# sim590/opendht

Measured on AMD Instinct MI355X. Metric: k=8 closest-node queries/sec at 100M-node table (1/8 GPU) + % HBM roofline, higher is better.
Workload: dtype u64

## Files before the change

opendht_amd/csrc/kad_swarm.hip:

```cpp
#include <hip/hip_runtime.h>

#include <algorithm>
#include <cstdlib>
#include <cstdarg>
#include <cstdint>
#include <cstdio>
#include <cstring>
#include <mutex>
#include <string>
#include <vector>

#include "../../include/kadgpu.h"

namespace kadgpu_internal {
int set_error(int code, const char* msg);
bool device_ok(int dev);
}

namespace {

constexpr uint32_t NONE = 0xFFFFFFFFu;
constexpr uint32_t L = KAD_SWARM_LEVELS;
constexpr uint32_t BK = 8;
constexpr uint32_t SN = 14;
// ... 197 lines not shown
    };
    const uint32_t lv = (uint32_t)(__builtin_bitreverse64(k) & ((1ull << D) - 1));
    const uint32_t m1 = lv, m0 = ~lv & (uint32_t)((1ull << D) - 1);
    const uint32_t M = (uint32_t)__builtin_popcount(m1), B = D + 1;
    const uint64_t x = k ^ t.hi;
    const uint32_t c = x ? (uint32_t)__builtin_clzll(x) : 64u;
    uint32_t b;
    if (c >= D) b = M;
    else if ((m1 >> c) & 1u) b = (uint32_t)__builtin_popcount(m1 & ((1u << c) - 1u));
    else b = M + 1 + (uint32_t)__builtin_popcount(m0 & ~((2u << c) - 1u));
    const uint32_t n0 = (uint32_t)__builtin_popcount(m0);
    auto level = [&](uint32_t P) -> uint32_t {
        if (P < M) return nth_bit(m1, P);
        if (P == M) return D;
        return nth_bit(m0, n0 - 1 - (P - M - 1));
    };
    uint32_t lo = b > 0 ? b - 1 : 0, hi = b, good = cnt(level(b)) + (b > 0 ? cnt(level(b - 1)) : 0u);
    while (good < count && !(lo == 0 && hi == B - 1)) {
        if (hi < B - 1) { hi++; good += cnt(level(hi)); }
        if (lo > 0) { lo--; good += cnt(level(lo)); }
    }
    uint64_t L0[K];
    uint32_t LI[K];
#pragma unroll
    for (uint32_t s = 0; s < K; s++) { L0[s] = ~0ull; LI[s] = NONE; }
    uint32_t nl = 0;
    uint64_t nin = ~0ull;
    bool tie = false;
    static_assert(!NET || K == BK, "the network ranks 8");
    static_assert(BK == 8, "a level's slots are four 16-byte key loads and one 16-byte index rule");
    struct Slots {
        uint64_t k[BK];
        uint4 rule;
        uint32_t nb;
    };
    auto load_level = [&](uint32_t P, Slots& S) {
        const uint32_t d = level(P);
        S.nb = cnt(d);
        const uint4* kp4 = reinterpret_cast<const uint4*>(W.lvl + ((size_t)p * L + d) * LVL_WORDS);
        S.rule = kp4[LVL_RULE / 4];
#pragma unroll
        for (int x = 0; x < 4; x++) {
            const uint4 u = kp4[x];
            S.k[2 * x] = ((uint64_t)u.y << 32) | u.x;
            S.k[2 * x + 1] = ((uint64_t)u.w << 32) | u.z;
        }
    };
    Slots cur, nxt;
    load_level(lo, cur);
    for (uint32_t P = lo; P <= hi; P++) {
        if (P < hi) load_level(P + 1, nxt);
        const uint32_t nb = cur.nb;
        const uint64_t* ek = cur.k;
        if constexpr (NET) {
            uint32_t ej[BK];
#pragma unroll
            for (uint32_t j = 0; j < BK; j++) {
                cur.k[j] = j < nb ? cur.k[j] ^ t.hi : ~0ull;
                ej[j] = j;
                tie |= j < nb && cur.k[j] == ~0ull;
            }
            sort8_kid(cur.k, ej);
#pragma unroll
            for (uint32_t s = 0; s < K; s++) {
                const bool sw = cur.k[K - 1 - s] < L0[s];
                nin = min(nin, sw ? L0[s] : cur.k[K - 1 - s]);
                L0[s] = sw ? cur.k[K - 1 - s] : L0[s];
                LI[s] = sw ? (cur.k[K - 1 - s] != ~0ull ? lvl_index(cur.rule, ej[K - 1 - s]) : NONE) : LI[s];
            }
#pragma unroll
            for (uint32_t h = K / 2; h >= 1; h >>= 1)
#pragma unroll
                for (uint32_t r = 0; r < K; r++)
                    if ((r & h) == 0) cx_kid(L0[r], LI[r], L0[r + h], LI[r + h]);
            nl = min(nl + nb, K);
            if (P < hi) cur = nxt;
            continue;
        }
        uint32_t ei[BK];
#pragma unroll
        for (uint32_t j = 0; j < BK; j++) ei[j] = lvl_index(cur.rule, j);
#pragma unroll 1
        for (uint32_t j = 0; j < nb; j++) {
            uint64_t cd = ek[0];
            uint32_t ci = ei[0];
#pragma unroll
            for (uint32_t y = 1; y < BK; y++) {
                cd = j == y ? ek[y] : cd;
                ci = j == y ? ei[y] : ci;
            }
            cd ^= t.hi;
            bool sh = false;
#pragma unroll
            for (uint32_t s = 0; s < K; s++) {
                const bool lt = sh || s >= nl || cd < L0[s] || (cd == L0[s] && tail_less(W, t, ci, LI[s]));
                sh = lt;
                const uint64_t n0_ = lt ? L0[s] : cd;
                const uint32_t n1_ = lt ? LI[s] : ci;
                if (lt) { L0[s] = cd; LI[s] = ci; }
                cd = n0_;
                ci = n1_;
            }
            nl = min(nl + 1, K);
        }
        if (P < hi) cur = nxt;
    }
    if constexpr (NET) {
#pragma unroll
        for (uint32_t s = 0; s + 1 < K; s++) tie |= L0[s] != ~0ull && L0[s] == L0[s + 1];
        tie |= nin != ~0ull && L0[K - 1] == nin;
        if (tie) return TIE;
    }
    const uint32_t m = min(nl, count);
#pragma unroll
    for (uint32_t s = 0; s < K; s++) {
        oi[s] = LI[s];
        ok[s] = L0[s] ^ t.hi;
    }
    return m;
}

__global__ __launch_bounds__(BLOCK) void swarm_closest_kernel(SwarmDev W, const uint32_t* peers, const uint8_t* targets, uint32_t q, uint32_t count,
                                     uint32_t* out_idx, uint8_t* out_cnt) {
    const uint32_t i = blockIdx.x * BLOCK + threadIdx.x;
    if (i >= q) return;
    uint32_t oi[SNP];
    uint64_t ok[SNP];
    const uint32_t p = peers[i];
    const uint32_t m = p < W.n ? peer_closest<SNP>(W, p, load_tgt(targets, i), count, oi, ok) : 0u;
    for (uint32_t s = 0; s < count; s++) out_idx[(size_t)i * count + s] = s < m ? oi[s] : NONE;
    if (out_cnt) out_cnt[i] = (uint8_t)m;
}

struct SearchDev {
    const uint32_t* src;
    const uint8_t* targets;
    uint32_t* li;
    uint64_t* lk;
    uint8_t* lq;
    uint8_t* lb;
    uint8_t* ln;
    uint32_t* hops;
    uint8_t* done;
    uint32_t* sel;
    uint32_t* ri;
    uint64_t* rk;
    uint8_t* rn;
    uint32_t* active;
    uint32_t* overflow;
    uint32_t* xo;
    uint8_t* xn;
    uint32_t S;
    uint32_t offline;
};

__device__ __forceinline__ uint64_t sw_mix(uint64_t x) {
    x += 0x9E3779B97F4A7C15ull;
    x = (x ^ (x >> 30)) * 0xBF58476D1CE4E5B9ull;
    x = (x ^ (x >> 27)) * 0x94D049BB133111EBull;
    return x ^ (x >> 31);
}

__device__ __forceinline__ bool swarm_offline(uint32_t p, uint32_t per10k) {
    return per10k && (uint32_t)(sw_mix((uint64_t)p * 0x9E37ull + 0xBADull) % 10000ull) < per10k;
}

__device__ __forceinline__ uint32_t lo_mask(uint32_t n) { return n >= 32 ? ~0u : (1u << n) - 1u; }

template <uint32_t N>
__device__ __forceinline__ void select_next(const SearchDev& X, uint32_t s, uint32_t n, uint32_t& qm, uint32_t bm,
                                            const uint32_t (&li)[N]) {
    uint32_t rest = ~(qm | bm) & lo_mask(min(n, N)), pick = 0;
#pragma unroll
    for (uint32_t a = 0; a < ALPHA; a++) {
        pick |= rest & (0u - rest);
        rest &= rest - 1u;
    }
    qm |= pick;
    uint32_t sel[ALPHA] = {NONE, NONE, NONE, NONE};
#pragma unroll
    for (uint32_t j = 0; j < N; j++) {
        const uint32_t rk = (uint32_t)__builtin_popcount(pick & ((1u << j) - 1u));
        if ((pick >> j) & 1u)
#pragma unroll
            for (uint32_t a = 0; a < ALPHA; a++)
                if (a == rk) sel[a] = li[j];
    }
    reinterpret_cast<uint4*>(X.sel)[s] = make_uint4(sel[0], sel[1], sel[2], sel[3]);
    if (!pick) X.done[s] = 2;
}

__device__ __forceinline__ uint32_t load_flags(const uint8_t* f, uint32_t s, uint32_t n = LST) {
    const uint4* p = reinterpret_cast<const uint4*>(f + (size_t)s * LST);
    uint32_t m = 0;
#pragma unroll
    for (int x = 0; x < (int)LST / 16; x++) {
        const uint4 u = 16u * x < n ? p[x] : make_uint4(0, 0, 0, 0);
        const uint32_t w[4] = {u.x, u.y, u.z, u.w};
#pragma unroll
        for (int y = 0; y < 4; y++)
#pragma unroll
            for (int z = 0; z < 4; z++) m |= (((w[y] >> (8 * z)) & 255u) ? 1u : 0u) << (16 * x + 4 * y + z);
    }
    return m;
}
__device__ __forceinline__ void store_flags(uint8_t* f, uint32_t s, uint32_t m, uint32_t n, uint32_t w = LST) {
    m &= lo_mask(n);
    uint4* p = reinterpret_cast<uint4*>(f + (size_t)s * LST);
#pragma unroll
    for (int x = 0; x < (int)LST / 16; x++) {
        if (16u * x >= w) continue;
        uint32_t w[4];
#pragma unroll
        for (int y = 0; y < 4; y++) {
            w[y] = 0;
#pragma unroll
            for (int z = 0; z < 4; z++) w[y] |= ((m >> (16 * x + 4 * y + z)) & 1u) << (8 * z);
        }
        p[x] = make_uint4(w[0], w[1], w[2], w[3]);
    }
}
static_assert(LST == 32 && ALPHA == 4, "the flag masks are 32 bits, the selection one 16-byte store");

__global__ __launch_bounds__(BLOCK) void search_init_kernel(SwarmDev W, SearchDev X) {
    const uint32_t s = blockIdx.x * BLOCK + threadIdx.x;
    if (s >= X.S) return;
    uint32_t li[SNP];
    uint64_t lk[SNP];
    uint32_t qm = 0;
    const uint32_t p = X.src[s];
    const uint32_t n = p < W.n ? peer_closest<SNP>(W, p, load_tgt(X.targets, s), SN, li, lk) : 0u;
    X.done[s] = n ? 0 : 2;
    X.hops[s] = 0;
    X.ln[s] = (uint8_t)n;
    if (n) select_next(X, s, n, qm, 0u, li);
#pragma unroll
    for (uint32_t j = 0; j < LST; j++) {
        X.li[(size_t)s * LST + j] = j < SNP && j < n ? li[j < SNP ? j : 0] : NONE;
        X.lk[(size_t)s * LST + j] = j < SNP && j < n ? lk[j < SNP ? j : 0] : ~0ull;
    }
    store_flags(X.lq, s, qm, n);
    store_flags(X.lb, s, 0u, n);
}

template <bool NET>
__global__ __launch_bounds__(BLOCK) __attribute__((amdgpu_waves_per_eu(SW_QUERY_WPE, 8))) void search_query_kernel(SwarmDev W, SearchDev X) {
    const uint32_t g = blockIdx.x * BLOCK + threadIdx.x;
    if (g >= X.S * ALPHA) return;
    const uint32_t s = g / ALPHA;
    const uint32_t sv = X.sel[g];
    const Tgt t = load_tgt(X.targets, s);
    const uint32_t v = X.done[s] ? NONE : sv;
    uint32_t oi[BK];
    uint64_t ok[BK];
    const bool up = v < W.n && !swarm_offline(v, X.offline);
    uint32_t m = up ? (NET ? peer_closest<BK, true>(W, v, t, BK, oi, ok) : TIE) : 0u;
    if (m == TIE) m = peer_closest<BK>(W, v, t, BK, oi, ok);
    if (m) {
        uint4* pi = reinterpret_cast<uint4*>(X.ri + (size_t)g * BK);
        uint4* pk = reinterpret_cast<uint4*>(X.rk + (size_t)g * BK);
#pragma unroll
        for (uint32_t x = 0; x < BK / 4; x++)
            if (4 * x < m) pi[x] = make_uint4(oi[4 * x], oi[4 * x + 1], oi[4 * x + 2], oi[4 * x + 3]);
#pragma unroll
        for (uint32_t x = 0; x < BK / 2; x++)
            if (2 * x < m)
                pk[x] = make_uint4((uint32_t)ok[2 * x], (uint32_t)(ok[2 * x] >> 32), (uint32_t)ok[2 * x + 1],
                                   (uint32_t)(ok[2 * x + 1] >> 32));
    }
    X.rn[g] = (uint8_t)m;
}

constexpr uint32_t XO_CAP = 64;

template <uint32_t N>
__device__ __forceinline__ void search_insert(const SwarmDev& W, const Tgt& t, uint32_t (&li)[N], uint64_t (&ld)[N],
                                              uint32_t& qm, uint32_t& bm, uint32_t& n, uint32_t r, uint64_t rd, bool rbad,
                                              bool& ovf) {
    bool found = false, anyeq = false;
    uint32_t pos = 0;
#pragma unroll
    for (uint32_t k = 0; k < N; k++) {
        if (k < n) {
            found |= li[k] == r;
            pos += ld[k] < rd;
            anyeq |= ld[k] == rd;
        }
    }
    if (found) return;
    uint32_t tie = 0;
    if (anyeq) {
#pragma unroll
        for (uint32_t k = 0; k < N; k++)
            if (k < n) tie |= (ld[k] == rd && li[k] != r ? 1u : 0u) << k;
    }
    while (tie) {
        const uint32_t k = (uint32_t)__builtin_ctz(tie);
        tie &= tie - 1u;
        uint32_t lk = 0;
#pragma unroll
        for (uint32_t x = 0; x < N; x++) lk = x == k ? li[x] : lk;
        pos += tail_less(W, t, lk, r);
    }
    uint32_t bad = (uint32_t)__builtin_popcount(bm & lo_mask(n));
    const bool full = n - bad >= SN;
    if (full) {
        uint32_t good = ~bm & lo_mask(n);
#pragma unroll
        for (uint32_t k = 0; k < SN; k++) good &= good - 1u;
        const uint32_t tt = good ? (uint32_t)__builtin_ctz(good) : n;
        n = tt;
        bad = (uint32_t)__builtin_popcount(bm & lo_mask(n));
        if (pos >= tt) return;
    }
    if (n == N) {
        bad -= (bm >> (N - 1)) & 1u;
        n--;
        ovf = true;
        if (pos >= n) return;
    }
#pragma unroll
    for (uint32_t k = N - 1; k > 0; k--) {
        li[k] = k > pos ? li[k - 1] : k == pos ? r : li[k];
        ld[k] = k > pos ? ld[k - 1] : k == pos ? rd : ld[k];
    }
    li[0] = pos == 0 ? r : li[0];
    ld[0] = pos == 0 ? rd : ld[0];
    const uint32_t low = lo_mask(pos), bit = 1u << pos;
    qm = (qm & low) | ((qm & ~low) << 1);
    bm = (bm & low) | ((bm & ~low) << 1) | (rbad ? bit : 0u);
    n++;
    bad += rbad ? 1u : 0u;
    if (n - bad > SN) {
        uint32_t good = ~bm & lo_mask(n);
#pragma unroll
        for (uint32_t k = 0; k < SN; k++) good &= good - 1u;
        n = (uint32_t)__builtin_ctz(good);
        bad = (uint32_t)__builtin_popcount(bm & lo_mask(n));
    }
}

struct Answers {
    uint32_t r[BK];
    uint64_t k[BK];
};
__device__ __forceinline__ void load_answers(const SearchDev& X, uint32_t g, uint32_t rn, Answers& A) {
    const uint4* pi = reinterpret_cast<const uint4*>(X.ri + (size_t)g * BK);
    const uint4* pk = reinterpret_cast<const uint4*>(X.rk + (size_t)g * BK);
#pragma unroll
    for (uint32_t x = 0; x < BK / 4; x++) {
        const uint4 u = 4 * x < rn ? pi[x] : make_uint4(NONE, NONE, NONE, NONE);
        A.r[4 * x] = u.x; A.r[4 * x + 1] = u.y; A.r[4 * x + 2] = u.z; A.r[4 * x + 3] = u.w;
    }
#pragma unroll
    for (uint32_t x = 0; x < BK / 2; x++) {
        const uint4 u = 2 * x < rn ? pk[x] : make_uint4(0, 0, 0, 0);
        A.k[2 * x] = ((uint64_t)u.y << 32) | u.x;
        A.k[2 * x + 1] = ((uint64_t)u.w << 32) | u.z;
    }
}

template <uint32_t N, bool FUSED>
__device__ __forceinline__ bool merge_lookup(const SwarmDev& W, const SearchDev& X, uint32_t s, uint32_t n0, uint32_t bm0,
                                             uint32_t xn) {
    {
        const Tgt t = load_tgt(X.targets, s);
        uint32_t li[N];
        uint64_t ld[N];
        uint32_t n = n0;
        const uint4 sv = reinterpret_cast<const uint4*>(X.sel)[s];
        const uint32_t sel[ALPHA] = {sv.x, sv.y, sv.z, sv.w};
        const uint32_t rn4 = FUSED ? 0u : *reinterpret_cast<const uint32_t*>(X.rn + (size_t)s * ALPHA);
        Answers A[2];
        if (!FUSED) load_answers(X, s * ALPHA, rn4 & 255u, A[0]);
        {
            const uint4* pi = reinterpret_cast<const uint4*>(X.li + (size_t)s * LST);
            const uint4* pk = reinterpret_cast<const uint4*>(X.lk + (size_t)s * LST);
#pragma unroll
            for (uint32_t x = 0; x < N / 4; x++) {
                const uint4 u = 4 * x < n0 ? pi[x] : make_uint4(NONE, NONE, NONE, NONE);
                li[4 * x] = u.x; li[4 * x + 1] = u.y; li[4 * x + 2] = u.z; li[4 * x + 3] = u.w;
            }
#pragma unroll
            for (uint32_t x = 0; x < N / 2; x++) {
                const uint4 u = 2 * x < n0 ? pk[x] : make_uint4(~0u, ~0u, ~0u, ~0u);
                ld[2 * x] = (((uint64_t)u.y << 32) | u.x) ^ t.hi;
                ld[2 * x + 1] = (((uint64_t)u.w << 32) | u.z) ^ t.hi;
            }
        }
        uint32_t qm = load_flags(X.lq, s, n0), bm = bm0;
        const uint32_t src = X.src[s];
        bool ovf = false;
        const uint32_t* xo = X.xo + (size_t)s * XO_CAP;
#pragma unroll
        for (uint32_t a = 0; a < ALPHA; a++) {
            uint32_t rn;
            if (FUSED) {
                const uint32_t v = sel[a];
                const bool up = v < W.n && !swarm_offline(v, X.offline);
                rn = up ? peer_closest<BK>(W, v, t, BK, A[a & 1].r, A[a & 1].k) : 0u;
            } else {
                if (a + 1 < ALPHA) load_answers(X, s * ALPHA + a + 1, (rn4 >> (8 * (a + 1))) & 255u, A[(a + 1) & 1]);
                rn = (rn4 >> (8 * a)) & 255u;
            }
            const Answers& C = A[a & 1];
            for (uint32_t j = 0; j < rn; j++) {
                uint32_t r = C.r[0];
                uint64_t rk = C.k[0];
#pragma unroll
                for (uint32_t x = 1; x < BK; x++) {
                    r = j == x ? C.r[x] : r;
                    rk = j == x ? C.k[x] : rk;
                }
                if (r == src) continue;
                bool rbad = false;
                if (swarm_offline(r, X.offline))
                    for (uint32_t e = 0; e < xn && !rbad; e++) rbad = xo[e] == r;
                search_insert(W, t, li, ld, qm, bm, n, r, rk ^ t.hi, rbad, ovf);
            }
        }
#pragma unroll
        for (uint32_t a = 0; a < ALPHA; a++) {
            const uint32_t v = sel[a];
            if (v == NONE || !swarm_offline(v, X.offline)) continue;
            if (xn < XO_CAP) X.xo[(size_t)s * XO_CAP + xn++] = v;
            else ovf = true;
#pragma unroll
            for (uint32_t k = 0; k < N; k++)
                if (k < n && li[k] == v) bm |= 1u << k;
        }
        X.xn[s] = (uint8_t)xn;
        X.hops[s] += 1;
        const uint32_t nm = lo_mask(n), good = ~bm & nm;
        uint32_t first8 = good;
        {
            uint32_t rest = good;
#pragma unroll
            for (uint32_t k = 0; k < BK; k++) rest &= rest - 1u;
            first8 &= ~rest;
        }
        const bool synced = (first8 & ~qm) == 0;
        const uint32_t lead = ~(bm & nm), cb = lead ? (uint32_t)__builtin_ctz(lead) : 32u;
        if (synced && first8) X.done[s] = 1;
        else if (n > 0 && cb >= min(n, MAX_BAD)) X.done[s] = 3;
        else select_next(X, s, n, qm, bm, li);
        X.ln[s] = (uint8_t)n;
        const uint32_t wn = max(n, n0);
        {
            uint4* pi = reinterpret_cast<uint4*>(X.li + (size_t)s * LST);
            uint4* pk = reinterpret_cast<uint4*>(X.lk + (size_t)s * LST);
#pragma unroll
            for (uint32_t x = 0; x < N / 4; x++)
                if (4 * x < wn)
                    pi[x] = make_uint4(4 * x < n ? li[4 * x] : NONE, 4 * x + 1 < n ? li[4 * x + 1] : NONE,
                                       4 * x + 2 < n ? li[4 * x + 2] : NONE, 4 * x + 3 < n ? li[4 * x + 3] : NONE);
#pragma unroll
            for (uint32_t x = 0; x < N / 2; x++) {
                if (2 * x >= wn) continue;
                const uint64_t k0 = 2 * x < n ? ld[2 * x] ^ t.hi : ~0ull, k1 = 2 * x + 1 < n ? ld[2 * x + 1] ^ t.hi : ~0ull;
                pk[x] = make_uint4((uint32_t)k0, (uint32_t)(k0 >> 32), (uint32_t)k1, (uint32_t)(k1 >> 32));
            }
        }
        store_flags(X.lq, s, qm, n, wn);
        store_flags(X.lb, s, bm, n, wn);
        if (ovf) atomicAdd(X.overflow, 1u);
        return !X.done[s];
    }
}

template <bool PF>
__device__ __forceinline__ bool merge_lookup_net(const SwarmDev& W, const SearchDev& X, uint32_t s) {
    constexpr uint32_t QB = 0x80000000u, IM = 0x7FFFFFFFu;
    const uint64_t MAXK = ~0ull;
    const Tgt t = load_tgt(X.targets, s);
    const uint32_t n0 = X.ln[s];
    uint32_t li[16];
    uint64_t lk[16];
    {
        const uint4* pi = reinterpret_cast<const uint4*>(X.li + (size_t)s * LST);
        const uint4* pk = reinterpret_cast<const uint4*>(X.lk + (size_t)s * LST);
#pragma unroll
        for (uint32_t x = 0; x < 4; x++) {
            const uint4 u = 4 * x < n0 ? pi[x] : make_uint4(NONE, NONE, NONE, NONE);
            li[4 * x] = u.x; li[4 * x + 1] = u.y; li[4 * x + 2] = u.z; li[4 * x + 3] = u.w;
        }
#pragma unroll
        for (uint32_t x = 0; x < 8; x++) {
            const uint4 u = 2 * x < n0 ? pk[x] : make_uint4(~0u, ~0u, ~0u, ~0u);
            lk[2 * x] = 2 * x < n0 ? (((uint64_t)u.y << 32) | u.x) ^ t.hi : MAXK;
            lk[2 * x + 1] = 2 * x + 1 < n0 ? (((uint64_t)u.w << 32) | u.z) ^ t.hi : MAXK;
        }
    }
    const uint32_t qm0 = load_flags(X.lq, s, n0);
#pragma unroll
    for (uint32_t k = 0; k < 16; k++)
        if (k < n0 && ((qm0 >> k) & 1u)) li[k] |= QB;
    const uint32_t rn4 = *reinterpret_cast<const uint32_t*>(X.rn + (size_t)s * ALPHA);
    const uint32_t src = X.src[s];
    bool tie = false;
#pragma unroll
    for (uint32_t k = 0; k + 1 < 16; k++) tie |= li[k + 1] != NONE && lk[k] == lk[k + 1];
    Answers A, An;
    if (PF) load_answers(X, s * ALPHA, rn4 & 255u, A);
#pragma unroll 1
    for (uint32_t a = 0; a < ALPHA; a++) {
        const uint32_t rn = (rn4 >> (8 * a)) & 255u;
        if (!PF) load_answers(X, s * ALPHA + a, rn, A);
        else if (a + 1 < ALPHA) load_answers(X, s * ALPHA + a + 1, (rn4 >> (8 * (a + 1))) & 255u, An);
        uint64_t bk[BK];
        uint32_t bi[BK];
#pragma unroll
        for (uint32_t j = 0; j < BK; j++) {
            const uint32_t r = A.r[j];
            bool drop = j >= rn || r == src;
#pragma unroll
            for (uint32_t k = 0; k < 16; k++) drop |= (li[k] & IM) == r;
            bk[j] = drop ? MAXK : A.k[j] ^ t.hi;
            bi[j] = drop ? NONE : r;
        }
        sort8_kid(bk, bi);
#pragma unroll
        for (uint32_t i = 8; i < 16; i++) {
            const bool sw = bk[15 - i] < lk[i];
            lk[i] = sw ? bk[15 - i] : lk[i];
            li[i] = sw ? bi[15 - i] : li[i];
        }
#pragma unroll
        for (uint32_t h = 8; h >= 1; h >>= 1)
#pragma unroll
            for (uint32_t r = 0; r < 16; r++)
                if ((r & h) == 0) cx_kid(lk[r], li[r], lk[r + h], li[r + h]);
#pragma unroll
        for (uint32_t k = 0; k + 1 < 16; k++) tie |= li[k + 1] != NONE && lk[k] == lk[k + 1];
        if (PF) A = An;
    }
    if (tie) {
        X.done[s] = 4;
        return false;
    }
    uint32_t n = 0, qm = 0;
#pragma unroll
    for (uint32_t k = 0; k < SN; k++) {
        n += li[k] != NONE ? 1u : 0u;
        qm |= (li[k] != NONE && (li[k] & QB)) ? 1u << k : 0u;
        li[k] = li[k] != NONE ? li[k] & IM : NONE;
    }
    X.hops[s] += 1;
    const uint32_t nm = lo_mask(n);
    uint32_t first8 = nm;
    {
        uint32_t rest = nm;
#pragma unroll
        for (uint32_t k = 0; k < BK; k++) rest &= rest - 1u;
        first8 &= ~rest;
    }
    const bool synced = (first8 & ~qm) == 0;
    if (synced && first8) X.done[s] = 1;
    else select_next(X, s, n, qm, 0u, li);
    X.ln[s] = (uint8_t)n;
    const uint32_t wn = max(n, n0);
    {
        uint4* pi = reinterpret_cast<uint4*>(X.li + (size_t)s * LST);
        uint4* pk = reinterpret_cast<uint4*>(X.lk + (size_t)s * LST);
#pragma unroll
        for (uint32_t x = 0; x < 4; x++)
            if (4 * x < wn)
                pi[x] = make_uint4(4 * x < n ? li[4 * x] : NONE, 4 * x + 1 < n ? li[4 * x + 1] : NONE,
                                   4 * x + 2 < n ? li[4 * x + 2] : NONE, 4 * x + 3 < n ? li[4 * x + 3] : NONE);
#pragma unroll
        for (uint32_t x = 0; x < 8; x++) {
            if (2 * x >= wn) continue;
            const uint64_t k0 = 2 * x < n ? lk[2 * x] ^ t.hi : ~0ull, k1 = 2 * x + 1 < n ? lk[2 * x + 1] ^ t.hi : ~0ull;
            pk[x] = make_uint4((uint32_t)k0, (uint32_t)(k0 >> 32), (uint32_t)k1, (uint32_t)(k1 >> 32));
        }
    }
    store_flags(X.lq, s, qm, n, wn);
    store_flags(X.lb, s, 0u, n, wn);
    return !X.done[s];
}

template <bool PF>
__global__ __launch_bounds__(BLOCK) void search_merge_net_kernel(SwarmDev W, SearchDev X) {
    const uint32_t s = blockIdx.x * BLOCK + threadIdx.x;
    const bool running = s < X.S && !X.done[s] && merge_lookup_net<PF>(W, X, s);
    const uint64_t m = __ballot(running);
    if ((threadIdx.x & 63u) == 0 && m) atomicAdd(X.active, (uint32_t)__builtin_popcountll(m));
}

template <bool FUSED, uint32_t N, bool RETRY = false>
__global__ __launch_bounds__(BLOCK) __attribute__((amdgpu_waves_per_eu(N == 16 ? SW_NARROW_WPE : 1, 8))) void search_merge_kernel(SwarmDev W, SearchDev X) {
    const uint32_t s = blockIdx.x * BLOCK + threadIdx.x;
    const bool live = s < X.S && X.done[s] == (RETRY ? 4u : 0u);
    if (RETRY && live) X.done[s] = 0;
    bool running = false;
    if (live) {
        const uint32_t n0 = X.ln[s];
        running = merge_lookup<N, FUSED>(W, X, s, n0, N == LST ? load_flags(X.lb, s, n0) : 0u, N == LST ? X.xn[s] : 0u);
    }
    const uint64_t m = __ballot(running);
    if ((threadIdx.x & 63u) == 0 && m) atomicAdd(X.active, (uint32_t)__builtin_popcountll(m));
}

}

struct SearchBufs {
    std::vector<void*> owned;
    SearchDev X{};
    uint32_t* src = nullptr;
    uint8_t* targets = nullptr;
    uint32_t cap = 0;
    void release() {
        for (void* p : owned) (void)hipFree(p);
        owned.clear();
        cap = 0;
    }
};
struct kad_swarm {
    int device = 0;
    SwarmDev W{};
    std::vector<void*> owned;
    uint64_t bytes = 0;
    mutable std::mutex pool_mu;
    mutable SearchBufs pool;
    ~kad_swarm() {
        pool.release();
        for (void* p : owned) (void)hipFree(p);
    }
};

struct kad_search {
    int device = 0;
    const kad_swarm* sw = nullptr;
    SearchDev X{};
    hipStream_t stream = nullptr;
    SearchBufs bufs;
    ~kad_search() { bufs.release(); }
};

namespace {
template <class T>
int alloc(T** p, size_t count, std::vector<void*>& owned, uint64_t* bytes = nullptr) {
    void* q = nullptr;
    const size_t nb = std::max<size_t>(count * sizeof(T), 16);
    hipError_t e = hipMalloc(&q, nb);
    if (e != hipSuccess) return err(KAD_ERR_NOMEM, "hipMalloc(%zu) failed: %s", nb, hipGetErrorString(e));
    owned.push_back(q);
    if (bytes) *bytes += nb;
    *p = static_cast<T*>(q);
    return KAD_OK;
}

struct Guard {
    int prev = -1;
    explicit Guard(int dev) {
        if (hipGetDevice(&prev) != hipSuccess) prev = -1;
        if (prev != dev) (void)hipSetDevice(dev);
    }
    ~Guard() {
        int cur;
        if (prev >= 0 && hipGetDevice(&cur) == hipSuccess && cur != prev) (void)hipSetDevice(prev);
    }
};
}

extern "C" {

int kad_swarm_create(kad_swarm** out, int device, uint32_t n, const uint8_t* sorted_ids) {
    if (!out || (n && !sorted_ids)) return err(KAD_ERR_INVALID, "NULL argument");
    *out = nullptr;
    if (n < 2) return err(KAD_ERR_INVALID, "a swarm needs at least 2 peers");
    if (!kadgpu_internal::device_ok(device)) return err(KAD_ERR_NO_DEVICE, "device %d is not a gfx950 GPU", device);
    std::vector<uint64_t> key(n);
    std::vector<uint32_t> tail(3ull * n);
    for (uint32_t i = 0; i < n; i++) {
        const uint8_t* p = sorted_ids + 20ull * i;
        uint64_t k = 0;
        for (int b = 0; b < 8; b++) k = (k << 8) | p[b];
        key[i] = k;
        for (int w = 0; w < 3; w++)
            tail[3ull * i + w] = ((uint32_t)p[8 + 4 * w] << 24) | ((uint32_t)p[9 + 4 * w] << 16) |
                                 ((uint32_t)p[10 + 4 * w] << 8) | p[11 + 4 * w];
        if (i && std::memcmp(sorted_ids + 20ull * (i - 1), p, 20) >= 0)
            return err(KAD_ERR_INVALID, "peer IDs must be strictly ascending (index %u)", i);
    }
    Guard g(device);
    kad_swarm* s = new kad_swarm;
    s->device = device;
    uint64_t* dk;
    uint32_t* dt;
    int rc;
    if ((rc = alloc(&dk, n, s->owned, &s->bytes)) || (rc = alloc(&dt, 3ull * n, s->owned, &s->bytes)) ||
        (rc = alloc(&s->W.hdr, (size_t)n * HDR_WORDS, s->owned, &s->bytes)) ||
        (rc = alloc(&s->W.lvl, (size_t)n * L * LVL_WORDS, s->owned, &s->bytes))) {
        delete s;
        return rc;
    }
    if (hipMemcpy(dk, key.data(), 8ull * n, hipMemcpyHostToDevice) != hipSuccess ||
        hipMemcpy(dt, tail.data(), 12ull * n, hipMemcpyHostToDevice) != hipSuccess) {
        delete s;
        return err(KAD_ERR_HIP, "upload failed");
    }
    s->W.key = dk;
    s->W.tail = dt;
    s->W.n = n;
    hipLaunchKernelGGL(swarm_build_kernel, dim3(grid_for(n)), dim3(BLOCK), 0, 0, s->W);
    if (hipGetLastError() != hipSuccess || hipDeviceSynchronize() != hipSuccess) {
        delete s;
        return err(KAD_ERR_HIP, "swarm table build failed");
    }
    *out = s;
    return KAD_OK;
}

int kad_swarm_destroy(kad_swarm* s) {
    if (!s) return KAD_OK;
    Guard g(s->device);
    (void)hipDeviceSynchronize();
    delete s;
    return KAD_OK;
}

int kad_swarm_info(const kad_swarm* s, uint32_t* n_peers, uint64_t* device_bytes) {
    if (!s) return err(KAD_ERR_INVALID, "NULL swarm");
    if (n_peers) *n_peers = s->W.n;
    if (device_bytes) *device_bytes = s->bytes;
    return KAD_OK;
}

int kad_swarm_get_table(const kad_swarm* s, uint32_t peer, uint32_t* depth, uint8_t* counts, uint32_t* entries) {
    if (!s || !depth || !counts || !entries) return err(KAD_ERR_INVALID, "NULL argument");
    if (peer >= s->W.n) return err(KAD_ERR_INVALID, "peer %u >= %u", peer, s->W.n);
    Guard g(s->device);
    uint32_t h[HDR_WORDS];
    std::vector<uint32_t> lv((size_t)L * LVL_WORDS);
    SW_TRY(hipMemcpy(h, s->W.hdr + (size_t)peer * HDR_WORDS, sizeof h, hipMemcpyDeviceToHost));
    SW_TRY(hipMemcpy(lv.data(), s->W.lvl + (size_t)peer * L * LVL_WORDS, 4 * lv.size(), hipMemcpyDeviceToHost));
    *depth = h[2];
    for (uint32_t d = 0; d < L; d++) {
        counts[d] = (uint8_t)(h[4 + d / 4] >> (8 * (d % 4)));
        for (uint32_t j = 0; j < BK; j++) entries[d * BK + j] = lv[(size_t)d * LVL_WORDS + LVL_IDX + j];
    }
    return KAD_OK;
}

int kad_swarm_closest_batch(const kad_swarm* s, const uint32_t* peers, const uint8_t* targets, uint32_t q,
                            uint32_t count, uint32_t* out_idx, uint8_t* out_cnt, void* stream) {
    if (!s) return err(KAD_ERR_INVALID, "NULL swarm");
    if (count > SNP) return err(KAD_ERR_UNSUPPORTED, "count %u > %u", count, SNP);
    if (q == 0) return KAD_OK;
    if (!peers || !targets || !out_idx) return err(KAD_ERR_INVALID, "NULL buffer");
    Guard g(s->device);
    hipLaunchKernelGGL(swarm_closest_kernel, dim3(grid_for(q)), dim3(BLOCK), 0, (hipStream_t)stream, s->W, peers,
                       targets, q, count, out_idx, out_cnt);
    SW_TRY(hipGetLastError());
    return KAD_OK;
}

int kad_search_create(kad_search** out, const kad_swarm* s, uint32_t S, const uint32_t* src, const uint8_t* targets,
                      uint32_t offline_per_10k, void* stream) {
    if (!out || !s || (S && (!src || !targets))) return err(KAD_ERR_INVALID, "NULL argument");
    *out = nullptr;
    Guard g(s->device);
    kad_search* x = new kad_search;
    x->device = s->device;
    x->sw = s;
    x->stream = (hipStream_t)stream;
    SearchDev& X = x->X;
    X.S = S;
    if (offline_per_10k > 10000) {
        delete x;
        return err(KAD_ERR_INVALID, "offline_per_10k %u > 10000", offline_per_10k);
    }
    X.offline = offline_per_10k;
    {
        std::lock_guard<std::mutex> lk(s->pool_mu);
        if (S && s->pool.cap >= S) std::swap(x->bufs, s->pool);
    }
    SearchBufs& B = x->bufs;
    if (!B.cap) {
        SearchDev& Y = B.X;
        std::vector<void*>& o = B.owned;
        const uint32_t C = S;
        int rc;
        if ((rc = alloc(&B.src, C, o)) || (rc = alloc(&B.targets, 20ull * C, o)) ||
            (rc = alloc(&Y.li, (size_t)C * LST, o)) || (rc = alloc(&Y.lk, (size_t)C * LST, o)) ||
            (rc = alloc(&Y.lq, (size_t)C * LST, o)) || (rc = alloc(&Y.lb, (size_t)C * LST, o)) ||
            (rc = alloc(&Y.ln, C, o)) || (rc = alloc(&Y.overflow, 1, o)) || (rc = alloc(&Y.hops, C, o)) ||
            (rc = alloc(&Y.done, C, o)) || (rc = alloc(&Y.sel, (size_t)C * ALPHA, o)) ||
            (rc = alloc(&Y.ri, (size_t)C * ALPHA * BK, o)) || (rc = alloc(&Y.rk, (size_t)C * ALPHA * BK, o)) ||
            (rc = alloc(&Y.rn, (size_t)C * ALPHA, o)) || (rc = alloc(&Y.active, 1, o)) ||
            (rc = alloc(&Y.xo, (size_t)C * XO_CAP, o)) || (rc = alloc(&Y.xn, C, o))) {
            delete x;
            return rc;
        }
        B.cap = std::max<uint32_t>(C, 1);
    }
    {
        const uint32_t S0 = X.S, off0 = X.offline;
        X = B.X;
        X.S = S0;
        X.offline = off0;
    }
    uint32_t* dsrc = B.src;
    uint8_t* dt = B.targets;
    if (S && (hipMemcpyAsync(dsrc, src, 4ull * S, hipMemcpyDefault, x->stream) != hipSuccess ||
              hipMemcpyAsync(dt, targets, 20ull * S, hipMemcpyDefault, x->stream) != hipSuccess)) {
        delete x;
        return err(KAD_ERR_HIP, "search upload failed");
    }
    X.src = dsrc;
    X.targets = dt;
    if (hipMemsetAsync(X.overflow, 0, 4, x->stream) != hipSuccess ||
        hipMemsetAsync(X.xn, 0, std::max<uint32_t>(S, 1), x->stream) != hipSuccess) {
        delete x;
        return err(KAD_ERR_HIP, "search init failed");
    }
    if (S) hipLaunchKernelGGL(search_init_kernel, dim3(grid_for(S)), dim3(BLOCK), 0, x->stream, s->W, X);
    if (hipGetLastError() != hipSuccess) {
        delete x;
        return err(KAD_ERR_HIP, "search init launch failed");
    }
    *out = x;
    return KAD_OK;
}

static bool narrow_off() {
    static const bool off = std::getenv("KAD_SWARM_WIDE") != nullptr;
    return off;
}

static bool net_off() {
    static const bool off = std::getenv("KAD_SWARM_SEQ") != nullptr;
    return off;
}

static bool net_pf_off() {
    static const bool off = [] {
        const char* e = std::getenv("KAD_SWARM_NETPF");
        return e && !std::strcmp(e, "0");
    }();
    return off;
}

static bool qnet_off() {
    static const bool off = [] {
        const char* e = std::getenv("KAD_SWARM_QUERY");
        return e && !std::strcmp(e, "ins");
    }();
    return off;
}

int kad_search_hop(kad_search* x, uint32_t* n_active) {
    if (!x) return err(KAD_ERR_INVALID, "NULL search");
    Guard g(x->device);
    const SearchDev& X = x->X;
    SW_TRY(hipMemsetAsync(X.active, 0, 4, x->stream));
    if (X.S) {
        static const bool split = std::getenv("KAD_SWARM_FUSED") == nullptr;
        if (split) {
            const dim3 qg(grid_for((uint64_t)X.S * ALPHA));
            if (qnet_off())
                hipLaunchKernelGGL(search_query_kernel<false>, qg, dim3(BLOCK), 0, x->stream, x->sw->W, X);
            else
                hipLaunchKernelGGL(search_query_kernel<true>, qg, dim3(BLOCK), 0, x->stream, x->sw->W, X);
            if (X.offline == 0 && !narrow_off() && !net_off()) {
                if (net_pf_off())
                    hipLaunchKernelGGL(search_merge_net_kernel<false>, dim3(grid_for(X.S)), dim3(BLOCK), 0, x->stream,
                                       x->sw->W, X);
                else
                    hipLaunchKernelGGL(search_merge_net_kernel<true>, dim3(grid_for(X.S)), dim3(BLOCK), 0, x->stream,
                                       x->sw->W, X);
                hipLaunchKernelGGL((search_merge_kernel<false, 16, true>), dim3(grid_for(X.S)), dim3(BLOCK), 0,
                                   x->stream, x->sw->W, X);
            } else if (X.offline == 0 && !narrow_off())
                hipLaunchKernelGGL((search_merge_kernel<false, 16>), dim3(grid_for(X.S)), dim3(BLOCK), 0, x->stream,
                                   x->sw->W, X);
            else
                hipLaunchKernelGGL((search_merge_kernel<false, LST>), dim3(grid_for(X.S)), dim3(BLOCK), 0, x->stream,
                                   x->sw->W, X);
        } else {
            hipLaunchKernelGGL((search_merge_kernel<true, LST>), dim3(grid_for(X.S)), dim3(BLOCK), 0, x->stream, x->sw->W, X);
        }
    }
    SW_TRY(hipGetLastError());
    if (n_active) {
        SW_TRY(hipMemcpyAsync(n_active, X.active, 4, hipMemcpyDeviceToHost, x->stream));
        SW_TRY(hipStreamSynchronize(x->stream));
    }
    return KAD_OK;
}

int kad_search_get(const kad_search* x, uint32_t* list, uint8_t* queried, uint8_t* bad, uint8_t* n, uint32_t* hops,
                   uint8_t* done, uint32_t* overflow) {
    if (!x) return err(KAD_ERR_INVALID, "NULL search");
    Guard g(x->device);
    const SearchDev& X = x->X;
    SW_TRY(hipStreamSynchronize(x->stream));
    const size_t S = X.S;
    if (list) SW_TRY(hipMemcpy(list, X.li, 4 * S * LST, hipMemcpyDeviceToHost));
    if (queried) SW_TRY(hipMemcpy(queried, X.lq, S * LST, hipMemcpyDeviceToHost));
    if (bad) SW_TRY(hipMemcpy(bad, X.lb, S * LST, hipMemcpyDeviceToHost));
    if (n) SW_TRY(hipMemcpy(n, X.ln, S, hipMemcpyDeviceToHost));
    if (hops) SW_TRY(hipMemcpy(hops, X.hops, 4 * S, hipMemcpyDeviceToHost));
    if (done) SW_TRY(hipMemcpy(done, X.done, S, hipMemcpyDeviceToHost));
    if (overflow) SW_TRY(hipMemcpy(overflow, X.overflow, 4, hipMemcpyDeviceToHost));
    return KAD_OK;
}

int kad_search_destroy(kad_search* x) {
    if (!x) return KAD_OK;
    Guard g(x->device);
    if (hipStreamSynchronize(x->stream) == hipSuccess && x->sw && x->bufs.cap) {
        std::lock_guard<std::mutex> lk(x->sw->pool_mu);
        if (x->bufs.cap > x->sw->pool.cap) std::swap(x->bufs, x->sw->pool);
    }
    delete x;
    return KAD_OK;
}

}
```

opendht_amd/swarm.py:

```python
from __future__ import annotations

import ctypes as C

import numpy as np

from ._lib import check, lib, ptr

LEVELS = 28
SEARCH_NODES = 14
SEARCH_LIST = 32


class Swarm:
    def __init__(self, sorted_ids, device: int = 0):
        ids = np.ascontiguousarray(sorted_ids, dtype=np.uint8).reshape(-1, 20)
        self.n = ids.shape[0]
        self.device = device
        h = C.c_void_p()
        check(lib().kad_swarm_create(C.byref(h), device, self.n, ptr(ids)), "kad_swarm_create")
        self._h = h

    def close(self):
        if getattr(self, "_h", None):
            lib().kad_swarm_destroy(self._h)
            self._h = None

    def __del__(self):
        try:
            self.close()
        except Exception:
            pass

    def __enter__(self):
        return self

    def __exit__(self, *a):
        self.close()

    def device_bytes(self) -> int:
        b = C.c_uint64()
        check(lib().kad_swarm_info(self._h, None, C.byref(b)), "kad_swarm_info")
        return b.value

    def table(self, p: int):
        d = C.c_uint32()
        cnt = np.zeros(LEVELS, np.uint8)
        ent = np.zeros((LEVELS, 8), np.uint32)
        check(lib().kad_swarm_get_table(self._h, p, C.byref(d), ptr(cnt), ptr(ent)), "kad_swarm_get_table")
        return d.value, cnt, ent

    def closest(self, peers, targets, count: int):
        import torch

        q = peers.shape[0]
        idx = torch.empty((q, count), dtype=torch.int32, device=peers.device)
        cnt = torch.empty((q,), dtype=torch.uint8, device=peers.device)
        s = C.c_void_p(torch.cuda.current_stream(peers.device).cuda_stream)
        check(lib().kad_swarm_closest_batch(self._h, ptr(peers), ptr(targets), q, count, ptr(idx), ptr(cnt), s),
              "kad_swarm_closest_batch")
        return idx, cnt

    def search(self, src, targets, offline_per_10k: int = 0) -> "Search":
        return Search(self, src, targets, offline_per_10k)


class Search:
    def __init__(self, swarm: Swarm, src, targets, offline_per_10k: int = 0):
        import torch

        self.S = src.shape[0]
        self.swarm = swarm
        h = C.c_void_p()
        s = C.c_void_p(torch.cuda.current_stream(swarm.device).cuda_stream)
        check(lib().kad_search_create(C.byref(h), swarm._h, self.S, ptr(src), ptr(targets), offline_per_10k, s),
              "kad_search_create")
        self._h = h

    def hop(self) -> int:
        a = C.c_uint32()
        check(lib().kad_search_hop(self._h, C.byref(a)), "kad_search_hop")
        return a.value

    def run(self, max_hops: int = 64) -> int:
        for h in range(max_hops):
            if self.hop() == 0:
                return h + 1
        return max_hops

    def get(self, full: bool = False):
        S = self.S
        lst = np.empty((S, SEARCH_LIST), np.uint32)
        q = np.empty((S, SEARCH_LIST), np.uint8)
        bad = np.empty((S, SEARCH_LIST), np.uint8)
        n = np.empty((S,), np.uint8)
        hops = np.empty((S,), np.uint32)
        done = np.empty((S,), np.uint8)
        ovf = C.c_uint32()
        check(lib().kad_search_get(self._h, ptr(lst), ptr(q), ptr(bad), ptr(n), ptr(hops), ptr(done), C.byref(ovf)),
              "kad_search_get")
        if full:
            return lst, q, bad, n, hops, done, ovf.value
        return lst[:, :SEARCH_NODES].copy(), q[:, :SEARCH_NODES].copy(), np.minimum(n, SEARCH_NODES), hops, done

    def close(self):
        if getattr(self, "_h", None):
            lib().kad_search_destroy(self._h)
            self._h = None

    def __del__(self):
        try:
            self.close()
        except Exception:
            pass
```

Measured before the change: 33.39 billion.

## Compact live searches into clean/dirty lists to skip finished ones per hop

Each kernel now writes the surviving search indices into double-buffered live lists using wave ballots and atomics. Clean searches go at the front of the list and dirty ones (offline peers, bad nodes, overflow) at the back. Later hops launch grids sized to the live counts, so the query and merge kernels only visit active searches. The fast net merge path now runs on the clean subset even when offline nodes are present, and the dirty subset goes to the full-width merge. The cost is extra atomics, indirect loads, and host-tracked counts that go stale when n_active is not read back.

```diff
diff --git a/opendht_amd/csrc/kad_swarm.hip b/opendht_amd/csrc/kad_swarm.hip
--- a/opendht_amd/csrc/kad_swarm.hip
+++ b/opendht_amd/csrc/kad_swarm.hip
@@ -373,7 +373,43 @@
     uint8_t* xn;
     uint32_t S;
     uint32_t offline;
+    const uint32_t* lin;
+    uint32_t* lout;
+    const uint32_t* cin;
+    uint32_t* cout;
 };
+
+enum : uint32_t { LIVE_CLEAN = 0, LIVE_DIRTY = 1, LIVE_ALL = 2 };
+__device__ __forceinline__ uint32_t live_lookup(const SearchDev& X, uint32_t g, uint32_t part) {
+    if (!X.lin) return g < X.S ? g : NONE;
+    const uint32_t nc = min(X.cin[0], X.S), nd = min(X.cin[1], X.S - nc);
+    if (part != LIVE_DIRTY) {
+        if (g < nc) return X.lin[g];
+        if (part == LIVE_CLEAN) return NONE;
+        g -= nc;
+    }
+    return g < nd ? X.lin[X.S - 1u - g] : NONE;
+}
+
+__device__ __forceinline__ void live_append(const SearchDev& X, uint32_t s, uint32_t cls) {
+    const uint64_t mc = __ballot(cls == 1u), md = __ballot(cls == 2u);
+    const uint32_t lane = threadIdx.x & 63u;
+    if (!X.lout) {
+        if (lane == 0 && (mc | md)) atomicAdd(X.cout, (uint32_t)__builtin_popcountll(mc | md));
+        return;
+    }
+    uint32_t bc = 0, bd = 0;
+    if (lane == 0) {
+        if (mc) bc = atomicAdd(X.cout, (uint32_t)__builtin_popcountll(mc));
+        if (md) bd = atomicAdd(X.cout + 1, (uint32_t)__builtin_popcountll(md));
+    }
+    bc = __shfl(bc, 0, 64);
+    bd = __shfl(bd, 0, 64);
+    const uint64_t m = cls == 1u ? mc : md;
+    const uint32_t at = (cls == 1u ? bc : bd) +
+                        __builtin_amdgcn_mbcnt_hi((uint32_t)(m >> 32), __builtin_amdgcn_mbcnt_lo((uint32_t)m, 0u));
+    if (cls && at < X.S) X.lout[cls == 1u ? at : X.S - 1u - at] = s;
+}
 
 __device__ __forceinline__ uint64_t sw_mix(uint64_t x) {
     x += 0x9E3779B97F4A7C15ull;
@@ -389,7 +425,7 @@
 __device__ __forceinline__ uint32_t lo_mask(uint32_t n) { return n >= 32 ? ~0u : (1u << n) - 1u; }
 
 template <uint32_t N>
-__device__ __forceinline__ void select_next(const SearchDev& X, uint32_t s, uint32_t n, uint32_t& qm, uint32_t bm,
+__device__ __forceinline__ bool select_next(const SearchDev& X, uint32_t s, uint32_t n, uint32_t& qm, uint32_t bm,
                                             const uint32_t (&li)[N]) {
     uint32_t rest = ~(qm | bm) & lo_mask(min(n, N)), pick = 0;
 #pragma unroll
@@ -409,6 +445,11 @@
     }
     reinterpret_cast<uint4*>(X.sel)[s] = make_uint4(sel[0], sel[1], sel[2], sel[3]);
     if (!pick) X.done[s] = 2;
+    bool silent = false;
+    if (X.offline)
+#pragma unroll
+        for (uint32_t a = 0; a < ALPHA; a++) silent |= sel[a] != NONE && swarm_offline(sel[a], X.offline);
+    return silent;
 }
 
 __device__ __forceinline__ uint32_t load_flags(const uint8_t* f, uint32_t s, uint32_t n = LST) {
@@ -445,30 +486,36 @@
 
 __global__ __launch_bounds__(BLOCK) void search_init_kernel(SwarmDev W, SearchDev X) {
     const uint32_t s = blockIdx.x * BLOCK + threadIdx.x;
-    if (s >= X.S) return;
-    uint32_t li[SNP];
-    uint64_t lk[SNP];
-    uint32_t qm = 0;
-    const uint32_t p = X.src[s];
-    const uint32_t n = p < W.n ? peer_closest<SNP>(W, p, load_tgt(X.targets, s), SN, li, lk) : 0u;
-    X.done[s] = n ? 0 : 2;
-    X.hops[s] = 0;
-    X.ln[s] = (uint8_t)n;
-    if (n) select_next(X, s, n, qm, 0u, li);
-#pragma unroll
-    for (uint32_t j = 0; j < LST; j++) {
-        X.li[(size_t)s * LST + j] = j < SNP && j < n ? li[j < SNP ? j : 0] : NONE;
-        X.lk[(size_t)s * LST + j] = j < SNP && j < n ? lk[j < SNP ? j : 0] : ~0ull;
-    }
-    store_flags(X.lq, s, qm, n);
-    store_flags(X.lb, s, 0u, n);
+    uint32_t cls = 0;
+    if (s < X.S) {
+        uint32_t li[SNP];
+        uint64_t lk[SNP];
+        uint32_t qm = 0;
+        const uint32_t p = X.src[s];
+        const uint32_t n = p < W.n ? peer_closest<SNP>(W, p, load_tgt(X.targets, s), SN, li, lk) : 0u;
+        X.done[s] = n ? 0 : 2;
+        X.hops[s] = 0;
+        X.ln[s] = (uint8_t)n;
+        if (n) {
+            const bool silent = select_next(X, s, n, qm, 0u, li);
+            if (qm) cls = silent ? 2u : 1u;
+        }
+#pragma unroll
+        for (uint32_t j = 0; j < LST; j++) {
+            X.li[(size_t)s * LST + j] = j < SNP && j < n ? li[j < SNP ? j : 0] : NONE;
+            X.lk[(size_t)s * LST + j] = j < SNP && j < n ? lk[j < SNP ? j : 0] : ~0ull;
+        }
+        store_flags(X.lq, s, qm, n);
+        store_flags(X.lb, s, 0u, n);
+    }
+    live_append(X, s, cls);
 }
 
 template <bool NET>
 __global__ __launch_bounds__(BLOCK) __attribute__((amdgpu_waves_per_eu(SW_QUERY_WPE, 8))) void search_query_kernel(SwarmDev W, SearchDev X) {
-    const uint32_t g = blockIdx.x * BLOCK + threadIdx.x;
-    if (g >= X.S * ALPHA) return;
-    const uint32_t s = g / ALPHA;
+    const uint32_t s = live_lookup(X, (blockIdx.x * BLOCK + threadIdx.x) / ALPHA, LIVE_ALL);
+    if (s >= X.S) return;
+    const uint32_t g = s * ALPHA + (threadIdx.x % ALPHA);
     const uint32_t sv = X.sel[g];
     const Tgt t = load_tgt(X.targets, s);
     const uint32_t v = X.done[s] ? NONE : sv;
@@ -582,7 +629,7 @@
 }
 
 template <uint32_t N, bool FUSED>
-__device__ __forceinline__ bool merge_lookup(const SwarmDev& W, const SearchDev& X, uint32_t s, uint32_t n0, uint32_t bm0,
+__device__ __forceinline__ uint32_t merge_lookup(const SwarmDev& W, const SearchDev& X, uint32_t s, uint32_t n0, uint32_t bm0,
                                              uint32_t xn) {
     {
         const Tgt t = load_tgt(X.targets, s);
@@ -662,9 +709,10 @@
         }
         const bool synced = (first8 & ~qm) == 0;
         const uint32_t lead = ~(bm & nm), cb = lead ? (uint32_t)__builtin_ctz(lead) : 32u;
+        bool silent = false;
         if (synced && first8) X.done[s] = 1;
         else if (n > 0 && cb >= min(n, MAX_BAD)) X.done[s] = 3;
-        else select_next(X, s, n, qm, bm, li);
+        else silent = select_next(X, s, n, qm, bm, li);
         X.ln[s] = (uint8_t)n;
         const uint32_t wn = max(n, n0);
         {
@@ -685,12 +733,13 @@
         store_flags(X.lq, s, qm, n, wn);
         store_flags(X.lb, s, bm, n, wn);
         if (ovf) atomicAdd(X.overflow, 1u);
-        return !X.done[s];
+        if (X.done[s]) return 0u;
+        return silent || (bm & nm) || xn ? 2u : 1u;
     }
 }
 
 template <bool PF>
-__device__ __forceinline__ bool merge_lookup_net(const SwarmDev& W, const SearchDev& X, uint32_t s) {
+__device__ __forceinline__ uint32_t merge_lookup_net(const SwarmDev& W, const SearchDev& X, uint32_t s) {
     constexpr uint32_t QB = 0x80000000u, IM = 0x7FFFFFFFu;
     const uint64_t MAXK = ~0ull;
     const Tgt t = load_tgt(X.targets, s);
@@ -757,7 +806,7 @@
     }
     if (tie) {
         X.done[s] = 4;
-        return false;
+        return 0u;
     }
     uint32_t n = 0, qm = 0;
 #pragma unroll
@@ -776,8 +825,9 @@
         first8 &= ~rest;
     }
     const bool synced = (first8 & ~qm) == 0;
+    bool silent = false;
     if (synced && first8) X.done[s] = 1;
-    else select_next(X, s, n, qm, 0u, li);
+    else silent = select_next(X, s, n, qm, 0u, li);
     X.ln[s] = (uint8_t)n;
     const uint32_t wn = max(n, n0);
     {
@@ -797,29 +847,28 @@
     }
     store_flags(X.lq, s, qm, n, wn);
     store_flags(X.lb, s, 0u, n, wn);
-    return !X.done[s];
+    if (X.done[s]) return 0u;
+    return silent ? 2u : 1u;
 }
 
 template <bool PF>
 __global__ __launch_bounds__(BLOCK) void search_merge_net_kernel(SwarmDev W, SearchDev X) {
-    const uint32_t s = blockIdx.x * BLOCK + threadIdx.x;
-    const bool running = s < X.S && !X.done[s] && merge_lookup_net<PF>(W, X, s);
-    const uint64_t m = __ballot(running);
-    if ((threadIdx.x & 63u) == 0 && m) atomicAdd(X.active, (uint32_t)__builtin_popcountll(m));
+    const uint32_t s = live_lookup(X, blockIdx.x * BLOCK + threadIdx.x, LIVE_CLEAN);
+    const uint32_t cls = s < X.S && !X.done[s] ? merge_lookup_net<PF>(W, X, s) : 0u;
+    live_append(X, s, cls);
 }
 
 template <bool FUSED, uint32_t N, bool RETRY = false>
-__global__ __launch_bounds__(BLOCK) __attribute__((amdgpu_waves_per_eu(N == 16 ? SW_NARROW_WPE : 1, 8))) void search_merge_kernel(SwarmDev W, SearchDev X) {
-    const uint32_t s = blockIdx.x * BLOCK + threadIdx.x;
+__global__ __launch_bounds__(BLOCK) __attribute__((amdgpu_waves_per_eu(N == 16 ? SW_NARROW_WPE : 1, 8))) void search_merge_kernel(SwarmDev W, SearchDev X, uint32_t part) {
+    const uint32_t s = live_lookup(X, blockIdx.x * BLOCK + threadIdx.x, part);
     const bool live = s < X.S && X.done[s] == (RETRY ? 4u : 0u);
     if (RETRY && live) X.done[s] = 0;
-    bool running = false;
+    uint32_t cls = 0;
     if (live) {
         const uint32_t n0 = X.ln[s];
-        running = merge_lookup<N, FUSED>(W, X, s, n0, N == LST ? load_flags(X.lb, s, n0) : 0u, N == LST ? X.xn[s] : 0u);
-    }
-    const uint64_t m = __ballot(running);
-    if ((threadIdx.x & 63u) == 0 && m) atomicAdd(X.active, (uint32_t)__builtin_popcountll(m));
+        cls = merge_lookup<N, FUSED>(W, X, s, n0, N == LST ? load_flags(X.lb, s, n0) : 0u, N == LST ? X.xn[s] : 0u);
+    }
+    live_append(X, s, cls);
 }
 
 }
@@ -829,6 +878,7 @@
     SearchDev X{};
     uint32_t* src = nullptr;
     uint8_t* targets = nullptr;
+    uint32_t* live[2] = {nullptr, nullptr};
     uint32_t cap = 0;
     void release() {
         for (void* p : owned) (void)hipFree(p);
@@ -855,6 +905,8 @@
     SearchDev X{};
     hipStream_t stream = nullptr;
     SearchBufs bufs;
+    bool compact = false;
+    uint32_t cur = 0, n_clean = 0, n_dirty = 0, n_live = 0;
     ~kad_search() { bufs.release(); }
 };
 
@@ -977,6 +1029,14 @@
     return KAD_OK;
 }
 
+static bool compact_off() {
+    static const bool off = [] {
+        const char* e = std::getenv("KAD_SWARM_COMPACT");
+        return e && !std::strcmp(e, "0");
+    }();
+    return off;
+}
+
 int kad_search_create(kad_search** out, const kad_swarm* s, uint32_t S, const uint32_t* src, const uint8_t* targets,
                       uint32_t offline_per_10k, void* stream) {
     if (!out || !s || (S && (!src || !targets))) return err(KAD_ERR_INVALID, "NULL argument");
@@ -1009,8 +1069,9 @@
             (rc = alloc(&Y.ln, C, o)) || (rc = alloc(&Y.overflow, 1, o)) || (rc = alloc(&Y.hops, C, o)) ||
             (rc = alloc(&Y.done, C, o)) || (rc = alloc(&Y.sel, (size_t)C * ALPHA, o)) ||
             (rc = alloc(&Y.ri, (size_t)C * ALPHA * BK, o)) || (rc = alloc(&Y.rk, (size_t)C * ALPHA * BK, o)) ||
-            (rc = alloc(&Y.rn, (size_t)C * ALPHA, o)) || (rc = alloc(&Y.active, 1, o)) ||
-            (rc = alloc(&Y.xo, (size_t)C * XO_CAP, o)) || (rc = alloc(&Y.xn, C, o))) {
+            (rc = alloc(&Y.rn, (size_t)C * ALPHA, o)) || (rc = alloc(&Y.active, 4, o)) ||
+            (rc = alloc(&Y.xo, (size_t)C * XO_CAP, o)) || (rc = alloc(&Y.xn, C, o)) ||
+            (rc = alloc(&B.live[0], C, o)) || (rc = alloc(&B.live[1], C, o))) {
             delete x;
             return rc;
         }
@@ -1031,7 +1092,12 @@
     }
     X.src = dsrc;
     X.targets = dt;
+    x->compact = !compact_off();
+    X.lin = nullptr;
+    X.lout = x->compact ? B.live[0] : nullptr;
+    X.cin = X.cout = X.active;
     if (hipMemsetAsync(X.overflow, 0, 4, x->stream) != hipSuccess ||
+        hipMemsetAsync(X.active, 0, 16, x->stream) != hipSuccess ||
         hipMemsetAsync(X.xn, 0, std::max<uint32_t>(S, 1), x->stream) != hipSuccess) {
         delete x;
         return err(KAD_ERR_HIP, "search init failed");
@@ -1041,6 +1107,7 @@
         delete x;
         return err(KAD_ERR_HIP, "search init launch failed");
     }
+    x->n_clean = x->n_dirty = x->n_live = S;
     *out = x;
     return KAD_OK;
 }
@@ -1074,39 +1141,60 @@
 int kad_search_hop(kad_search* x, uint32_t* n_active) {
     if (!x) return err(KAD_ERR_INVALID, "NULL search");
     Guard g(x->device);
-    const SearchDev& X = x->X;
-    SW_TRY(hipMemsetAsync(X.active, 0, 4, x->stream));
-    if (X.S) {
+    SearchDev X = x->X;
+    uint32_t nc = X.S, nd = 0, nl = X.S;
+    if (x->compact) {
+        X.lin = x->bufs.live[x->cur];
+        X.lout = x->bufs.live[x->cur ^ 1u];
+        X.cin = X.active + 2u * x->cur;
+        X.cout = X.active + 2u * (x->cur ^ 1u);
+        nc = x->n_clean, nd = x->n_dirty, nl = x->n_live;
+        SW_TRY(hipMemsetAsync(X.cout, 0, 8, x->stream));
+    } else {
+        SW_TRY(hipMemsetAsync(X.active, 0, 4, x->stream));
+    }
+    const SwarmDev& W = x->sw->W;
+    const dim3 blk(BLOCK);
+    if (nl) {
         static const bool split = std::getenv("KAD_SWARM_FUSED") == nullptr;
+        const bool net = !narrow_off() && !net_off();
+        const dim3 ag(grid_for(nl));
         if (split) {
-            const dim3 qg(grid_for((uint64_t)X.S * ALPHA));
+            const dim3 qg(grid_for((uint64_t)nl * ALPHA));
             if (qnet_off())
-                hipLaunchKernelGGL(search_query_kernel<false>, qg, dim3(BLOCK), 0, x->stream, x->sw->W, X);
+                hipLaunchKernelGGL(search_query_kernel<false>, qg, blk, 0, x->stream, W, X);
             else
-                hipLaunchKernelGGL(search_query_kernel<true>, qg, dim3(BLOCK), 0, x->stream, x->sw->W, X);
-            if (X.offline == 0 && !narrow_off() && !net_off()) {
-                if (net_pf_off())
-                    hipLaunchKernelGGL(search_merge_net_kernel<false>, dim3(grid_for(X.S)), dim3(BLOCK), 0, x->stream,
-                                       x->sw->W, X);
-                else
-                    hipLaunchKernelGGL(search_merge_net_kernel<true>, dim3(grid_for(X.S)), dim3(BLOCK), 0, x->stream,
-                                       x->sw->W, X);
-                hipLaunchKernelGGL((search_merge_kernel<false, 16, true>), dim3(grid_for(X.S)), dim3(BLOCK), 0,
-                                   x->stream, x->sw->W, X);
+                hipLaunchKernelGGL(search_query_kernel<true>, qg, blk, 0, x->stream, W, X);
+            if (net && (X.offline == 0 || x->compact)) {
+                const dim3 cg(grid_for(nc));
+                if (nc) {
+                    if (net_pf_off())
+                        hipLaunchKernelGGL(search_merge_net_kernel<false>, cg, blk, 0, x->stream, W, X);
+                    else
+                        hipLaunchKernelGGL(search_merge_net_kernel<true>, cg, blk, 0, x->stream, W, X);
+                    hipLaunchKernelGGL((search_merge_kernel<false, 16, true>), cg, blk, 0, x->stream, W, X, LIVE_CLEAN);
+                }
+                if (nd)
+                    hipLaunchKernelGGL((search_merge_kernel<false, LST>), dim3(grid_for(nd)), blk, 0, x->stream, W, X,
+                                       LIVE_DIRTY);
             } else if (X.offline == 0 && !narrow_off())
-                hipLaunchKernelGGL((search_merge_kernel<false, 16>), dim3(grid_for(X.S)), dim3(BLOCK), 0, x->stream,
-                                   x->sw->W, X);
+                hipLaunchKernelGGL((search_merge_kernel<false, 16>), ag, blk, 0, x->stream, W, X, LIVE_ALL);
             else
-                hipLaunchKernelGGL((search_merge_kernel<false, LST>), dim3(grid_for(X.S)), dim3(BLOCK), 0, x->stream,
-                                   x->sw->W, X);
+                hipLaunchKernelGGL((search_merge_kernel<false, LST>), ag, blk, 0, x->stream, W, X, LIVE_ALL);
         } else {
-            hipLaunchKernelGGL((search_merge_kernel<true, LST>), dim3(grid_for(X.S)), dim3(BLOCK), 0, x->stream, x->sw->W, X);
+            hipLaunchKernelGGL((search_merge_kernel<true, LST>), ag, blk, 0, x->stream, W, X, LIVE_ALL);
         }
     }
     SW_TRY(hipGetLastError());
+    if (x->compact) x->cur ^= 1u;
     if (n_active) {
-        SW_TRY(hipMemcpyAsync(n_active, X.active, 4, hipMemcpyDeviceToHost, x->stream));
+        uint32_t len[2] = {0, 0};
+        SW_TRY(hipMemcpyAsync(len, X.cout, x->compact ? 8 : 4, hipMemcpyDeviceToHost, x->stream));
         SW_TRY(hipStreamSynchronize(x->stream));
+        *n_active = len[0] + len[1];
+        if (x->compact) x->n_clean = len[0], x->n_dirty = len[1], x->n_live = len[0] + len[1];
+    } else if (x->compact) {
+        x->n_clean = x->n_dirty = x->n_live;
     }
     return KAD_OK;
 }
diff --git a/opendht_amd/swarm.py b/opendht_amd/swarm.py
--- a/opendht_amd/swarm.py
+++ b/opendht_amd/swarm.py
@@ -1,6 +1,7 @@
 from __future__ import annotations
 
 import ctypes as C
+import weakref
 
 import numpy as np
 
@@ -19,9 +20,12 @@
         h = C.c_void_p()
         check(lib().kad_swarm_create(C.byref(h), device, self.n, ptr(ids)), "kad_swarm_create")
         self._h = h
+        self._searches = weakref.WeakSet()
 
     def close(self):
         if getattr(self, "_h", None):
+            for x in list(self._searches):
+                x.close()
             lib().kad_swarm_destroy(self._h)
             self._h = None
 
@@ -75,6 +79,7 @@
         check(lib().kad_search_create(C.byref(h), swarm._h, self.S, ptr(src), ptr(targets), offline_per_10k, s),
               "kad_search_create")
         self._h = h
+        swarm._searches.add(self)
 
     def hop(self) -> int:
         a = C.c_uint32()
@@ -106,6 +111,7 @@
         if getattr(self, "_h", None):
             lib().kad_search_destroy(self._h)
             self._h = None
+            self.swarm._searches.discard(self)
 
     def __del__(self):
         try:
```

Result: no change. 33.15 billion (-0.7%).
